# ucuapps/OpenGlue

Hardware: NVIDIA H100
Metric: image-pairs/sec at N=M=2048, d=256, 9 GNN layers, 100 Sinkhorn iters (higher is better)
Workload: dtype fp16x3 (fp16 hi/lo operands with power-of-two tensor scales, 3 products, fp32 accumulate)

## Files before the change

include/openglue_b200.h:

```cpp
#ifndef OPENGLUE_B200_H_
#define OPENGLUE_B200_H_

#include <stdint.h>

#ifdef __cplusplus
extern "C" {
#endif

#define OG_VERSION 100

typedef enum og_status {
  OG_OK = 0,
  OG_EINVAL = -1,
  OG_EUNSUPPORTED = -2,
  OG_ECUDA = -3,
  OG_EWORKSPACE = -4
} og_status;

typedef enum og_precision {
  OG_PREC_FP32 = 0,
  OG_PREC_TF32X3 = 1,
  OG_PREC_FP16X3 = 2
} og_precision;

// ... 74 lines not shown
  const float* R;  int64_t ldr;  int64_t strideR;
  const float* rscale;
  float* Y;  int64_t ldy;  int64_t strideY;
  float* Yt; int64_t ldyt; int64_t strideYt;
} og_linear_args;
int og_linear_fwd(const og_linear_args* args, int precision, void* stream);
int og_linear_tc_fwd(const og_linear_args* args, const float* Whi, const float* Wlo,
                     float* Yhi, float* Ylo, float* Ythi, float* Ytlo, int mode, void* stream);

int og_attention_fwd(const float* q, int64_t ldq, int64_t strideq,
                     const float* k, int64_t ldk, int64_t stridek,
                     const float* v, int64_t ldv, int64_t stridev,
                     float* out, int64_t ldo, int64_t strideo,
                     int batch, int nq, int nk, int num_heads, int head_dim,
                     int precision, void* stream);

int og_attention_tc_fwd(const float* q, int64_t ldq, int64_t strideq,
                        const float* khi, const float* klo, int64_t ldk,
                        const float* vthi, const float* vtlo, int64_t ldvt,
                        float* out, int64_t ldo, int64_t strideo,
                        int batch, int nq, int nk, int num_heads, int head_dim, void* stream);

int og_weight_split_f16(const float* w, const float* bias, int rows, int cols, void* hi16, void* lo16, float* meta, void* stream);
int og_amax(const float* x, int64_t n, float* slot, void* stream);
int og_linear_f16_fwd(const og_linear_args* args, const void* Wh16, const void* Wl16, const float* w_meta, const float* a_amax,
                      float* amax_out, float* scale_out, void* Yh, void* Yl, void* Yth, void* Ytl, int swap_halves, void* stream);
int og_attention_f16_fwd(const float* q, int64_t ldq, int64_t strideq, const float* q_amax,
                         const void* khi, const void* klo, int64_t ldk, const float* k_scale,
                         const void* vthi, const void* vtlo, int64_t ldvt, const float* v_scale,
                         float* out, int64_t ldo, int64_t strideo, float* out_amax,
                         int batch, int nq, int nk, int num_heads, int head_dim, int swap_halves, void* stream);

int64_t og_sinkhorn_workspace_bytes(int batch, int n, int m);
int og_sinkhorn_fwd(const float* S, int64_t lds, int64_t strideS, const float* dustbin,
                    int batch, int n, int m, int iters, float reg,
                    float* scores, void* workspace, int64_t workspace_bytes, void* stream);

int64_t og_sinkhorn_hist_floats(int batch, int n, int m, int iters);
int og_sinkhorn_train_fwd(const float* S, int64_t lds, int64_t strideS, const float* dustbin,
                          int batch, int n, int m, int iters, float reg, float* scores, float* hist,
                          void* workspace, int64_t workspace_bytes, void* stream);
int64_t og_sinkhorn_bwd_workspace_bytes(int batch, int n, int m, int iters);
int og_sinkhorn_bwd(const float* S, int64_t lds, int64_t strideS, const float* dustbin,
                    int batch, int n, int m, int iters, float reg, const float* hist,
                    const float* dscores, float* dS_aug, float* ddustbin,
                    void* workspace, int64_t workspace_bytes, void* stream);

int64_t og_match_workspace_bytes(int batch, int n, int m);
int og_match_fwd(const float* scores, int batch, int n, int m, float threshold,
                 int64_t* matches0, float* mscores0, int64_t* matches1, float* mscores1,
                 void* workspace, int64_t workspace_bytes, void* stream);

enum { OG_GT_PERSPECTIVE = 0, OG_GT_3D_REPROJECTION = 1 };
typedef struct og_gt_transform {
  int32_t type;
  const float* H;
  const float* K0; const float* K1;
  const float* R;  const float* T;
  const float* depth0;
  const float* depth1;
  int32_t depth_is_image;
  int32_t depth0_h, depth0_w, depth1_h, depth1_w;
} og_gt_transform;

int64_t og_gt_matches_workspace_bytes(int batch, int n, int m);
int og_gt_matches_fwd(const float* kpts0, const float* kpts1, int batch, int n, int m, const og_gt_transform* tf,
// ... 83 lines not shown
```

openglue_b200/_cabi.py:

```python
from __future__ import annotations

import ctypes as C
import os
from typing import Optional

import torch

_HERE = os.path.dirname(os.path.abspath(__file__))
LIB_PATH = os.path.join(_HERE, 'libopenglue_b200.so')

OG_OK = 0
OG_PREC_FP32, OG_PREC_TF32X3, OG_PREC_FP16X3 = 0, 1, 2
OG_MAX_HIDDEN = 8
(OG_T_KENC_W, OG_T_KENC_B, OG_T_QKV_W, OG_T_QKV_B, OG_T_FC1_W, OG_T_FC1_B, OG_T_FC2_W, OG_T_FC2_B,
 OG_T_PROJ_W, OG_T_PROJ_B, OG_T_PROJ_RMIX, OG_T_DUSTBIN) = range(12)


class OgConfig(C.Structure):
    _fields_ = [('descriptor_dim', C.c_int32), ('num_heads', C.c_int32), ('num_layers', C.c_int32),
                ('side_info_size', C.c_int32), ('num_hidden', C.c_int32), ('hidden', C.c_int32 * OG_MAX_HIDDEN),
                ('sinkhorn_iters', C.c_int32), ('sinkhorn_reg', C.c_float), ('match_threshold', C.c_float),
                ('precision', C.c_int32), ('no_descriptors', C.c_int32)]


# ... 17 lines not shown
    _fields_ = [('type', C.c_int32), ('H', C.c_void_p), ('K0', C.c_void_p), ('K1', C.c_void_p), ('R', C.c_void_p),
                ('T', C.c_void_p), ('depth0', C.c_void_p), ('depth1', C.c_void_p), ('depth_is_image', C.c_int32),
                ('depth0_h', C.c_int32), ('depth0_w', C.c_int32), ('depth1_h', C.c_int32), ('depth1_w', C.c_int32)]


OG_GT_PERSPECTIVE, OG_GT_3D_REPROJECTION = 0, 1

SYMBOLS = {
    'og_version': (_I, []),
    'og_last_error': (C.c_char_p, []),
    'og_device_info': (_I, [C.POINTER(C.c_int)] * 3),
    'og_packed_weight_floats': (_L, [_CFG]),
    'og_packed_offset': (_L, [_CFG, _I, _I]),
    'og_workspace_bytes': (_L, [_CFG, _I, _I, _I]),
    'og_split_tf32': (_I, [_P, _P, _P, _L, _P]),
    'og_linear_tc_fwd': (_I, [C.POINTER(OgLinearArgs), _P, _P, _P, _P, _P, _P, _I, _P]),
    'og_superglue_forward': (_I, [_CFG, _P, _P, _P, _I, _I, _I, _P, _P, _P, _P, _P, _P, C.POINTER(C.c_float),
                                  _P, _P, _P, _P, _P, _P, _P, _P, _L, _P]),
    'og_superglue_forward_f16': (_I, [_CFG, _P, _P, _P, _P, _P, _P, _I, _I, _I, _P, _P, _P, _P, _P, _P, C.POINTER(C.c_float),
                                      _P, _P, _P, _P, _P, _P, _P, _P, _L, _P]),
    'og_f16_meta_floats': (_L, [_CFG]),
    'og_pack_f16': (_I, [_CFG, _P, _P, _P, _P, _P]),
    'og_weight_split_f16': (_I, [_P, _P, _I, _I, _P, _P, _P, _P]),
    'og_amax': (_I, [_P, _L, _P, _P]),
    'og_linear_f16_fwd': (_I, [C.POINTER(OgLinearArgs), _P, _P, _P, _P, _P, _P, _P, _P, _P, _P, _I, _P]),
    'og_attention_f16_fwd': (_I, [_P, _L, _L, _P, _P, _P, _L, _P, _P, _P, _L, _P, _P, _L, _L, _P, _I, _I, _I, _I, _I, _I, _P]),
    'og_last_forward_launches': (_I, []),
    'og_set_tuning': (_I, [_I, _I]),
    'og_set_fusion': (_I, [_I]),
    'og_linear_fwd': (_I, [C.POINTER(OgLinearArgs), _I, _P]),
    'og_attention_fwd': (_I, [_P, _L, _L, _P, _L, _L, _P, _L, _L, _P, _L, _L, _I, _I, _I, _I, _I, _I, _P]),
    'og_attention_tc_fwd': (_I, [_P, _L, _L, _P, _P, _L, _P, _P, _L, _P, _L, _L, _I, _I, _I, _I, _I, _P]),
    'og_sinkhorn_workspace_bytes': (_L, [_I, _I, _I]),
    'og_sinkhorn_fwd': (_I, [_P, _L, _L, _P, _I, _I, _I, _I, _F, _P, _P, _L, _P]),
    'og_sinkhorn_hist_floats': (_L, [_I, _I, _I, _I]),
    'og_sinkhorn_train_fwd': (_I, [_P, _L, _L, _P, _I, _I, _I, _I, _F, _P, _P, _P, _L, _P]),
    'og_sinkhorn_bwd_workspace_bytes': (_L, [_I, _I, _I, _I]),
    'og_sinkhorn_bwd': (_I, [_P, _L, _L, _P, _I, _I, _I, _I, _F, _P, _P, _P, _P, _P, _L, _P]),
    'og_match_workspace_bytes': (_L, [_I, _I, _I]),
    'og_match_fwd': (_I, [_P, _I, _I, _I, _F, _P, _P, _P, _P, _P, _L, _P]),
    'og_gt_matches_workspace_bytes': (_L, [_I, _I, _I]),
    'og_collate_fwd': (_I, [_P, _P, _P, _P, _P, _I, _P, _I, _I, _P, _I, _I, _I, _I, _I, _P, _P, _P, _P, _P, _P, _P, _P, _P]),
    'og_criterion_workspace_bytes': (_L, [_I]),
    'og_criterion_fwd': (_I, [_P, _P, _P, _I, _I, _I, _P, _P, _F, _P, _L, _P]),
    'og_gt_matches_fwd': (_I, [_P, _P, _I, _I, _I, C.POINTER(OgGtTransform), _P, _P, _P, _L, _P]),
    'og_train_workspace_floats': (_L, [_I]),
    'og_linear_auto_scratch_floats': (_L, [C.POINTER(OgLinearArgs)]),
    'og_linear_auto_fwd': (_I, [C.POINTER(OgLinearArgs), _I, _P, _P]),
    'og_transpose': (_I, [_P, _L, _L, _P, _L, _L, _I, _I, _I, _I, _P]),
    'og_colsum': (_I, [_P, _L, _P, _L, _P, _L, _I, _I, _P, _P, _P]),
    'og_bn_train_fwd': (_I, [_P, _L, _I, _I, _I, _P, _P, _F, _F, _P, _L, _P, _P, _P, _P, _P, _P]),
    'og_bn_train_bwd': (_I, [_P, _L, _P, _L, _I, _I, _I, _P, _P, _P, _P, _L, _P, _P, _P, _P]),
    'og_softmax_rows': (_I, [_P, _L, _L, _I, _P]),
    'og_softmax_bwd_rows': (_I, [_P, _P, _L, _L, _I, _F, _P]),
    'og_axpby': (_I, [_P, _P, _F, _F, _P, _L, _P]),
    'og_sum_batches': (_I, [_P, _I, _I, _I, _P, _L, _I, _P]),
    'og_mix_fwd': (_I, [_P, _P, _P, _P, _L, _I, _P]),
    'og_mix_bwd': (_I, [_P, _P, _P, _P, _L, _I, _P]),
    'og_mix_param_grad': (_I, [_P, _P, _P, _I, _P]),
    'og_kenc_input': (_I, [_P, _P, _I, _I, _F, _F, _P, _P]),
    'og_sp_im2col3x3': (_I, [_P, _I, _I, _I, _I, _P, _P]),
    'og_sp_maxpool2x2': (_I, [_P, _I, _I, _I, _I, _P, _P]),
    'og_row_normalize': (_I, [_P, _L, _I, _I, _F, _P]),
    'og_sp_heat_nms': (_I, [_P, _I, _I, _I, _I, _F, _I, _P, _P]),
    'og_sp_compact': (_I, [_P, _I, _I, _I, _P, _P, _P, _P]),
    'og_sp_select': (_I, [_P, _P, _P, _P, _P, _I, _I, _I, _I, _I, _P, _P, _P]),
# ... 74 lines not shown
```

openglue_b200/csrc/api.cu:

```cuda
#include "common.cuh"
#include "linear_simt.cuh"
#include "linear_sm90.cuh"
#include "attention_simt.cuh"
#include "attention_sm90.cuh"
#include "sinkhorn.cuh"
#include "sinkhorn_bwd.cuh"
#include "match.cuh"
#include "gt_matches.cuh"
#include "criterion.cuh"
#include "collate.cuh"
#include "train_ops.cuh"
#include "superpoint.cuh"
#include "features.cuh"
#include "homography.cuh"
#include "optim.cuh"
#include <math.h>
#include <string.h>
#include <vector>

namespace og {

__global__ void __launch_bounds__(256) kenc_input_kernel(const float* __restrict__ kpts, const float* __restrict__ side,
                                                          int rows, int S, float wm1, float hm1, float* __restrict__ out) {
  const int r = blockIdx.x * blockDim.x + threadIdx.x;
// ... 271 lines not shown
  }
  return linear_simt_launch(*a, st);
}

int og_split_tf32(const float* src, float* hi, float* lo, int64_t n, void* stream) {
  OG_CHECK_ARG(src && hi && lo && n > 0, "split_tf32: bad arguments");
  return OG_LAUNCH(split_tf32_kernel, (unsigned)((n + 255) / 256), 256, 0, (cudaStream_t)stream, src, hi, lo, n);
}

int og_attention_fwd(const float* q, int64_t ldq, int64_t strideq, const float* k, int64_t ldk, int64_t stridek,
                     const float* v, int64_t ldv, int64_t stridev, float* out, int64_t ldo, int64_t strideo,
                     int batch, int nq, int nk, int num_heads, int head_dim, int precision, void* stream) {
  OG_CHECK_ARG(q && k && v && out, "attention: null pointer");
  OG_CHECK_ARG(batch > 0 && nq > 0 && nk > 0 && num_heads > 0 && head_dim > 0, "attention: bad sizes");
  (void)precision;
  AttnArgs a{q, ldq, strideq, k, ldk, stridek, v, ldv, stridev, out, ldo, strideo, batch, nq, nk, num_heads,
             (float)pow((double)head_dim, -0.5)};
  return attention_simt_launch(a, head_dim, (cudaStream_t)stream);
}

int og_attention_tc_fwd(const float* q, int64_t ldq, int64_t strideq, const float* khi, const float* klo, int64_t ldk,
                        const float* vthi, const float* vtlo, int64_t ldvt, float* out, int64_t ldo, int64_t strideo,
                        int batch, int nq, int nk, int num_heads, int head_dim, void* stream) {
  OG_CHECK_ARG(q && khi && klo && vthi && vtlo && out, "attention_tc: null pointer");
  OG_CHECK_ARG(batch > 0 && nq > 0 && nk > 0 && num_heads > 0, "attention_tc: bad sizes");
  if (!attention_tc_eligible(head_dim, ldq, ldk, ldvt, ldo))
    return fail(OG_EUNSUPPORTED, "attention_tc: head_dim in {32, 64} and 16-byte aligned rows required");
  TcAttnArgs a{q, ldq, strideq, out, ldo, strideo, batch, nq, nk, num_heads, num_heads * head_dim,
               (float)pow((double)head_dim, -0.5)};
  return attention_tc_launch(a, khi, klo, ldk, vthi, vtlo, ldvt, head_dim, (cudaStream_t)stream);
}

int64_t og_sinkhorn_workspace_bytes(int batch, int n, int m) { return sinkhorn_workspace_bytes(batch, n, m); }

int og_sinkhorn_fwd(const float* S, int64_t lds, int64_t strideS, const float* dustbin, int batch, int n, int m,
                    int iters, float reg, float* scores, void* workspace, int64_t workspace_bytes, void* stream) {
  OG_CHECK_ARG(S && dustbin && scores && workspace, "sinkhorn: null pointer");
  OG_CHECK_ARG(batch > 0 && n > 0 && m > 0 && iters >= 0 && reg > 0.f, "sinkhorn: bad sizes");
  return sinkhorn_launch(S, lds, strideS, dustbin, batch, n, m, iters, reg, scores, workspace, workspace_bytes,
                         (cudaStream_t)stream);
}

int64_t og_sinkhorn_hist_floats(int batch, int n, int m, int iters) {
  return (batch > 0 && n > 0 && m > 0 && iters >= 0) ? sinkhorn_hist_floats(batch, n, m, iters) : -1;
}

int og_sinkhorn_train_fwd(const float* S, int64_t lds, int64_t strideS, const float* dustbin, int batch, int n, int m,
                          int iters, float reg, float* scores, float* hist, void* workspace, int64_t workspace_bytes, void* stream) {
  OG_CHECK_ARG(S && dustbin && scores && workspace && hist, "sinkhorn_train_fwd: null pointer");
  OG_CHECK_ARG(batch > 0 && n > 0 && m > 0 && iters >= 0 && reg > 0.f, "sinkhorn_train_fwd: bad sizes");
  return sinkhorn_launch(S, lds, strideS, dustbin, batch, n, m, iters, reg, scores, workspace, workspace_bytes, (cudaStream_t)stream,
                         hist, hist + (int64_t)batch * iters * (n + 1));
}

int64_t og_sinkhorn_bwd_workspace_bytes(int batch, int n, int m, int iters) {
  return (batch > 0 && n > 0 && m > 0 && iters >= 0) ? sinkhorn_bwd_workspace_bytes(batch, n, m, iters) : -1;
}

int og_sinkhorn_bwd(const float* S, int64_t lds, int64_t strideS, const float* dustbin, int batch, int n, int m, int iters, float reg,
                    const float* hist, const float* dscores, float* dS_aug, float* ddustbin, void* workspace, int64_t workspace_bytes,
                    void* stream) {
  OG_CHECK_ARG(S && dustbin && hist && dscores && dS_aug && ddustbin && workspace, "sinkhorn_bwd: null pointer");
  OG_CHECK_ARG(batch > 0 && n > 0 && m > 0 && iters >= 0 && reg > 0.f, "sinkhorn_bwd: bad sizes");
  return sinkhorn_bwd_launch(S, lds, strideS, dustbin, batch, n, m, iters, reg, hist, dscores, dS_aug, ddustbin, workspace,
                             workspace_bytes, (cudaStream_t)stream);
}
// ... 595 lines not shown
```

openglue_b200/csrc/sinkhorn.cuh:

```cuda
#pragma once
#include "common.cuh"
#include "tc_common.cuh"
#include <math_constants.h>
#include <algorithm>

namespace og {

struct SinkArgs {
  static constexpr bool kBackward = false;
  const float* S; int64_t lds, strideS;
  const float* dustbin;
  int B, n, m, iters;
  float reg;
  float norm, log_a_last, log_b_last;
  float* scores;
  float* u;
  float* partial;
  unsigned int* barrier;
  int SP, rows_per_strip, mpad;
  float* hist_u;
  float* hist_v;
};

constexpr int SINK_WARPS = 8;
constexpr int64_t SINK_BARRIER_BYTES = 256 * 128;
constexpr int SINK_MAX_COLS = 8192;
constexpr int SINK_MAX_STRIPS = 32;
constexpr float LOG2E_F = 1.4426950408889634f;

__device__ __forceinline__ void grid_barrier(unsigned int* counter, unsigned int target) {
  __syncthreads();
  if (threadIdx.x == 0) {
    __threadfence();
    atomicAdd(counter, 1u);
    unsigned int seen;
    do {
      asm volatile("ld.acquire.gpu.global.u32 %0, [%1];" : "=r"(seen) : "l"(counter) : "memory");
    } while (seen < target);
    __threadfence();
  }
  __syncthreads();
}

typedef unsigned long long f32x2;
__device__ __forceinline__ f32x2 pk2(float x, float y) { f32x2 r; asm("mov.b64 %0, {%1, %2};" : "=l"(r) : "f"(x), "f"(y)); return r; }
__device__ __forceinline__ void upk2(f32x2 v, float& x, float& y) { asm("mov.b64 {%0, %1}, %2;" : "=f"(x), "=f"(y) : "l"(v)); }
#define OG_F32X2_OP(name, expr)                                        \
  __device__ __forceinline__ f32x2 name(f32x2 a, f32x2 b) {            \
    float ax, ay, bx, by; upk2(a, ax, ay); upk2(b, bx, by);            \
    auto op = [](float u, float v) { return expr; };                   \
    return pk2(op(ax, bx), op(ay, by));                                \
  }
// ... 100 lines not shown
        float4 q = (c < m) ? src[idx] : make_float4(0.f, 0.f, 0.f, 0.f);
        if (c < m && c + 3 >= m) {
          if (c + 1 >= m) q.y = 0.f;
          if (c + 2 >= m) q.z = 0.f;
          q.w = 0.f;
        }
        z[k] = q;
      }
    }
    ++consumed;
    __syncwarp();
    const int nxt = row + SLOTS * G;
    if (lane == 0 && nxt < end_real) copy(sl, nxt);
    if (a.reg != 1.0f) {
      const float reg = a.reg;
#pragma unroll
      for (int k = 0; k < V; ++k) {
        z[k].x = __fdiv_rn(z[k].x, reg); z[k].y = __fdiv_rn(z[k].y, reg);
        z[k].z = __fdiv_rn(z[k].z, reg); z[k].w = __fdiv_rn(z[k].w, reg);
      }
    }
  }
};

template <int V, int W, class X>
__device__ __forceinline__ const X* sink_row_exchange(X* xr, X mine, const SinkStrip<V, W>& s, uint32_t& rowpar) {
  X* x = xr + (rowpar * SinkStrip<V, W>::G + s.grp) * W;
  if (s.lane == 0) x[s.sub] = mine;
  asm volatile("bar.sync %0, %1;" ::"r"(1 + s.grp), "n"(W * 32) : "memory");
  rowpar ^= 1u;
  return x;
}

template <int V, int W, class Args, class Update>
__device__ __forceinline__ void sink_column_reduce(const Args& a, const SinkStrip<V, W>& s, float* red, const float4 (&cacc)[V],
                                                   float cacc_m, int k, Update update) {
  const int m = a.m;
  float* myred = red + s.grp * a.mpad;
#pragma unroll
  for (int q = 0; q < V; ++q) {
    const int c = s.c0 + 4 * (s.lane + 32 * q);
    if (c < m) *reinterpret_cast<float4*>(myred + c) = cacc[q];
  }
  __syncthreads();
  if (s.sub == 0 && s.lane == 0) myred[m] = cacc_m;
  __syncthreads();
  const int64_t buf = (int64_t)(k & 1) * a.B * a.SP + (int64_t)s.b * a.SP;
  float* part = a.partial + (buf + s.strip) * a.mpad;
  for (int j = s.tid; j <= m; j += blockDim.x) {
    float sum = 0.f;
#pragma unroll
    for (int w = 0; w < SinkStrip<V, W>::G; ++w) sum += red[w * a.mpad + j];
    part[j] = sum;
  }
  grid_barrier(a.barrier + 32 * s.b, (unsigned int)(k + 1) * (unsigned int)a.SP);
  const float* pb = a.partial + buf * a.mpad;
  for (int j4 = s.tid; 4 * j4 <= m; j4 += blockDim.x) {
    float4 c = make_float4(0.f, 0.f, 0.f, 0.f);
#pragma unroll 8
    for (int sp = 0; sp < a.SP; ++sp) {
      const float4 q = __ldcg(reinterpret_cast<const float4*>(pb + (int64_t)sp * a.mpad) + j4);
      c.x += q.x; c.y += q.y; c.z += q.z; c.w += q.w;
    }
    const float cc[4] = {c.x, c.y, c.z, c.w};
#pragma unroll
    for (int e = 0; e < 4; ++e) {
      const int j = 4 * j4 + e;
      if (j < m) update(j, cc[e]);
      else if (j == m) update(SinkStrip<V, W>::MC, cc[e]);
    }
  }
  __syncthreads();
}

template <int V, int W, int SLOTS>
__global__ void __launch_bounds__(SINK_WARPS * 32, (V <= 8) ? 2 : 1) sinkhorn_kernel(SinkArgs a) {
  extern __shared__ __align__(128) float og_sink_smem[];
  using Strip = SinkStrip<V, W>;
  constexpr int C = Strip::C, MC = Strip::MC, G = Strip::G;
  float* v_s = og_sink_smem;
  float* red = og_sink_smem + MC + 4;
  float* ring = red + G * a.mpad;
  uint64_t* bars = reinterpret_cast<uint64_t*>(ring + SINK_WARPS * SLOTS * C);
  float2* xr = reinterpret_cast<float2*>(bars + SINK_WARPS * SLOTS);
  const Strip s(a);
  const int n = a.n, m = a.m, c0 = s.c0, lane = s.lane, sub = s.sub;
  const float a_reg = expf(a.norm), a_last = expf(a.log_a_last);
  SinkRowRing<V, W, SLOTS, true, SinkArgs> rows(a, s, ring, bars);
  const float dz = rows.dz;

  for (int j = s.tid; j < MC; j += blockDim.x) v_s[j] = (j < m) ? 0.f : -CUDART_INF_F;
  if (s.tid == 0) v_s[MC] = 0.f;
  __syncthreads();

  rows.prime();
  uint32_t rowpar = 0;
  const f32x2 log2e2 = pk2(LOG2E_F, LOG2E_F);
  for (int it = 0; it < a.iters; ++it) {
    f32x2 cacc[2 * V];
#pragma unroll
    for (int k = 0; k < 2 * V; ++k) cacc[k] = 0ull;
    float cacc_m = 0.f;
    const float v_m = v_s[MC];

    for (int row = s.r0 + s.grp; row < s.r1; row += G) {
      float4 q[V];
      rows.take(row, q);
      f32x2 z[2 * V];
#pragma unroll
      for (int k = 0; k < V; ++k) { z[2 * k] = pk2(q[k].x, q[k].y); z[2 * k + 1] = pk2(q[k].z, q[k].w); }
      const float t_m = dz + v_m;
      float mx = (sub == 0) ? t_m : -CUDART_INF_F;
#pragma unroll
      for (int k = 0; k < V; ++k) {
        const ulonglong2 vv = *reinterpret_cast<const ulonglong2*>(v_s + c0 + 4 * (lane + 32 * k));
        z[2 * k] = add2(z[2 * k], vv.x); z[2 * k + 1] = add2(z[2 * k + 1], vv.y);
        float x0, x1, x2, x3; upk2(z[2 * k], x0, x1); upk2(z[2 * k + 1], x2, x3);
        mx = fmaxf(mx, fmaxf(fmaxf(x0, x1), fmaxf(x2, x3)));
      }
      mx = warp_max(mx);
      const float mxs = (mx == -CUDART_INF_F) ? 0.f : mx;
      const f32x2 mxs2 = pk2(mxs, mxs);
      f32x2 sum2a = 0ull, sum2b = 0ull;
#pragma unroll
      for (int k = 0; k < 2 * V; ++k) {
        float x, y; upk2(mul2(sub2(z[k], mxs2), log2e2), x, y);
        z[k] = pk2(ex2_approx(x), ex2_approx(y));
        if (k & 1) sum2b = add2(sum2b, z[k]); else sum2a = add2(sum2a, z[k]);
      }
      float sa, sb; upk2(add2(sum2a, sum2b), sa, sb);
      const float e_m = (sub == 0) ? ex2_approx((t_m - mxs) * LOG2E_F) : 0.f;
      float s_i = warp_sum(sa + sb) + e_m;
      float mxg = mx, f_w = 1.f;
      if (W > 1) {
        const float2* x = sink_row_exchange(xr, make_float2(mx, s_i), s, rowpar);
        float2 p[W];
#pragma unroll
        for (int w2 = 0; w2 < W; ++w2) { p[w2] = x[w2]; mxg = fmaxf(mxg, p[w2].x); }
        s_i = 0.f;
#pragma unroll
        for (int w2 = 0; w2 < W; ++w2) s_i = fmaf(p[w2].y, ex2_approx((p[w2].x - mxg) * LOG2E_F), s_i);
        f_w = ex2_approx((mx - mxg) * LOG2E_F);
      }
      const float w_i = __fdiv_rn((row < n) ? a_reg : a_last, s_i) * f_w;
      if ((it == a.iters - 1 || a.hist_u) && sub == 0 && lane == 0) {
        const float u_i = ((row < n) ? a.norm : a.log_a_last) - (mxg + logf(s_i));
        if (it == a.iters - 1) a.u[(int64_t)s.b * (n + 1) + row] = u_i;
        if (a.hist_u) a.hist_u[((int64_t)s.b * a.iters + it) * (n + 1) + row] = u_i;
      }
      const f32x2 w2 = pk2(w_i, w_i);
#pragma unroll
      for (int k = 0; k < 2 * V; ++k) cacc[k] = fma2(z[k], w2, cacc[k]);
      cacc_m = fmaf(e_m, w_i, cacc_m);
    }
    rows.prime();
    float4 c4[V];
#pragma unroll
    for (int k = 0; k < V; ++k) { upk2(cacc[2 * k], c4[k].x, c4[k].y); upk2(cacc[2 * k + 1], c4[k].z, c4[k].w); }
    sink_column_reduce(a, s, red, c4, cacc_m, it, [&](int j, float c) {
      v_s[j] = ((j < MC) ? a.norm : a.log_b_last) + v_s[j] - logf(c);
    });
    if (a.hist_v && s.strip == 0) {
      float* hv = a.hist_v + ((int64_t)s.b * (a.iters + 1) + it + 1) * (m + 1);
      for (int j = s.tid; j <= m; j += blockDim.x) hv[j] = (j < m) ? v_s[j] : v_s[MC];
    }
  }

  {
    const float v_m = v_s[MC];
    for (int row = s.r0 + s.grp; row < s.r1; row += G) {
      float4 z[V];
      rows.take(row, z);
      float u_i = 0.f;
      if (a.iters > 0) {
        if (lane == 0) u_i = __ldcg(a.u + (int64_t)s.b * (n + 1) + row);
        u_i = __shfl_sync(0xffffffffu, u_i, 0);
      }
      float* out = a.scores + ((int64_t)s.b * (n + 1) + row) * (m + 1);
#pragma unroll
      for (int k = 0; k < V; ++k) {
        const int c = c0 + 4 * (lane + 32 * k);
        if (c < m) {
          const float4 vv = *reinterpret_cast<const float4*>(v_s + c);
          if (c + 0 < m) out[c + 0] = (z[k].x + u_i) + vv.x - a.norm;
          if (c + 1 < m) out[c + 1] = (z[k].y + u_i) + vv.y - a.norm;
          if (c + 2 < m) out[c + 2] = (z[k].z + u_i) + vv.z - a.norm;
          if (c + 3 < m) out[c + 3] = (z[k].w + u_i) + vv.w - a.norm;
        }
      }
      if (sub == 0 && lane == 0) out[m] = (dz + u_i) + v_m - a.norm;
    }
  }
}

struct SinkPlan { int V, W, slots, occ, SP, rows_per_strip, mpad, pairs_per_launch; size_t smem; };

constexpr size_t sinkhorn_smem(bool backward, int V, int W, int slots, int mpad) {
  const int C = 128 * V, G = SINK_WARPS / W, vecs = backward ? 3 : 1;
  const size_t xbytes = backward ? sizeof(float) : sizeof(float2);
  return ((size_t)vecs * (W * C + 4) + (size_t)G * mpad + (size_t)SINK_WARPS * slots * C) * sizeof(float) +
         (size_t)SINK_WARPS * slots * sizeof(uint64_t) + (size_t)2 * G * W * xbytes + 128;
}

inline int sinkhorn_plan(bool backward, int B, int n, int m, SinkPlan* p) {
  const char* who = backward ? "sinkhorn_bwd" : "sinkhorn";
  if (m <= 512)                { p->V = 4;  p->W = 1; p->slots = 2; }
  else if (m <= 1024)          { p->V = 4;  p->W = 2; p->slots = 2; }
  else if (m <= 2048)          { p->V = 8;  p->W = 2; p->slots = 2; }
  else if (m <= 4096)          { p->V = 16; p->W = 2; p->slots = backward ? 1 : 2; }
  else if (m <= SINK_MAX_COLS) { p->V = 16; p->W = 4; p->slots = 1; }
  else return fail(OG_EUNSUPPORTED, "%s: m = %d > %d columns not supported (swap the images)", who, m, SINK_MAX_COLS);
  p->mpad = (int)align_up(m + 1, 4);
  p->smem = sinkhorn_smem(backward, p->V, p->W, p->slots, p->mpad);
  p->occ = (p->V <= 8 && 2 * (p->smem + 1024) <= OG_SMEM_OPTIN_MAX) ? 2 : 1;
  const int sms = device_info().ok ? device_info().sm_count : 132;
  const int ctas = sms * p->occ;
  p->pairs_per_launch = std::min(B < ctas ? B : ctas, (int)(SINK_BARRIER_BYTES / 128));
  int sp = std::min(ctas / p->pairs_per_launch, SINK_MAX_STRIPS);
  const int max_sp = cdiv(n + 1, SINK_WARPS / p->W);
  if (sp > max_sp) sp = max_sp;
  if (sp < 1) sp = 1;
  p->SP = sp;
  p->rows_per_strip = cdiv(n + 1, sp);
  return OG_OK;
}

inline int sinkhorn_check_rows(const char* who, const float* S, int64_t lds, int64_t strideS, int m) {
  if (lds % 4 != 0 || lds < m || !aligned16(S) || strideS % 4 != 0)
    return fail(OG_EINVAL, "%s: S rows must be 16-byte aligned (lds %% 4 == 0, lds >= m)", who);
  return OG_OK;
}

struct SinkConsts { float norm, log_a_last, log_b_last; };
inline SinkConsts sinkhorn_consts(int n, int m) {
  const float norm = -logf((float)(n + m));
  return {norm, norm + (float)log((double)m),
          norm + (float)log((double)n)};
}

template <auto Kernel, int V, int W, int SLOTS, class Args>
inline int sinkhorn_coop_launch(const Args& a, const SinkPlan& p, cudaStream_t stream) {
  constexpr size_t smem_max = sinkhorn_smem(Args::kBackward, V, W, SLOTS, 128 * V * W + 4);
  static_assert(smem_max <= OG_SMEM_OPTIN_MAX, "Sinkhorn kernel: shared memory beyond what one block may opt in to");
  if (const int rc = smem_opt_in<Kernel>((int)smem_max)) return rc;
  return launch(Args::kBackward ? "sinkhorn_bwd_kernel" : "sinkhorn_kernel", Kernel, LaunchAttr::cooperative, dim3(a.B * a.SP),
                dim3(SINK_WARPS * 32), p.smem, stream, a);
}

template <class Launch>
inline int sinkhorn_for_each_launch(const SinkPlan& p, int B, unsigned int* barrier, cudaStream_t stream, Launch&& launch) {
  for (int b0 = 0; b0 < B; b0 += p.pairs_per_launch) {
    const int nb = std::min(p.pairs_per_launch, B - b0);
    OG_CUDA(cudaMemsetAsync(barrier, 0, (size_t)nb * 128, stream));
    if (const int rc = launch(b0, nb)) return rc;
  }
  return OG_OK;
}

inline int64_t sinkhorn_workspace_bytes(int B, int n, int m) {
  SinkPlan p;
  if (sinkhorn_plan(false, B, n, m, &p) != OG_OK) return -1;
  return SINK_BARRIER_BYTES + align_up((int64_t)B * (n + 1) * 4, 256) + align_up(2LL * B * SINK_MAX_STRIPS * p.mpad * 4, 256);
}

inline int sinkhorn_launch(const float* S, int64_t lds, int64_t strideS, const float* dustbin, int B, int n, int m,
                           int iters, float reg, float* scores, void* ws, int64_t ws_bytes, cudaStream_t stream,
                           float* hist_u = nullptr, float* hist_v = nullptr) {
  SinkPlan p;
  if (const int rc = sinkhorn_plan(false, B, n, m, &p)) return rc;
  if (ws_bytes < sinkhorn_workspace_bytes(B, n, m)) return fail(OG_EWORKSPACE, "sinkhorn: workspace too small");
  if (const int rc = sinkhorn_check_rows("sinkhorn", S, lds, strideS, m)) return rc;
  char* w = static_cast<char*>(ws);
  unsigned int* barrier = reinterpret_cast<unsigned int*>(w); w += SINK_BARRIER_BYTES;
  float* u = reinterpret_cast<float*>(w); w += align_up((int64_t)B * (n + 1) * 4, 256);
  float* partial = reinterpret_cast<float*>(w);
  const SinkConsts k = sinkhorn_consts(n, m);
  if (hist_v) OG_CUDA(cudaMemsetAsync(hist_v, 0, (size_t)B * (iters + 1) * (m + 1) * sizeof(float), stream));
  return sinkhorn_for_each_launch(p, B, barrier, stream, [&](int b0, int nb) {
    SinkArgs a;
    a.S = S + (int64_t)b0 * strideS; a.lds = lds; a.strideS = strideS; a.dustbin = dustbin;
    a.B = nb; a.n = n; a.m = m; a.iters = iters; a.reg = reg;
    a.norm = k.norm; a.log_a_last = k.log_a_last; a.log_b_last = k.log_b_last;
    a.scores = scores + (int64_t)b0 * (n + 1) * (m + 1);
    a.u = u; a.partial = partial; a.barrier = barrier;
    a.SP = p.SP; a.rows_per_strip = p.rows_per_strip; a.mpad = p.mpad;
    a.hist_u = hist_u ? hist_u + (int64_t)b0 * iters * (n + 1) : nullptr;
    a.hist_v = hist_v ? hist_v + (int64_t)b0 * (iters + 1) * (m + 1) : nullptr;
    if (p.V == 4 && p.W == 1) return sinkhorn_coop_launch<sinkhorn_kernel<4, 1, 2>, 4, 1, 2>(a, p, stream);
    if (p.V == 4)             return sinkhorn_coop_launch<sinkhorn_kernel<4, 2, 2>, 4, 2, 2>(a, p, stream);
    if (p.V == 8)             return sinkhorn_coop_launch<sinkhorn_kernel<8, 2, 2>, 8, 2, 2>(a, p, stream);
    if (p.W == 2)             return sinkhorn_coop_launch<sinkhorn_kernel<16, 2, 2>, 16, 2, 2>(a, p, stream);
    return sinkhorn_coop_launch<sinkhorn_kernel<16, 4, 1>, 16, 4, 1>(a, p, stream);
  });
}

}
```

Before: 465.4.

## Add resident Sinkhorn kernel holding score rows on-chip with tagged flag exchange

Adds a Sinkhorn forward kernel that keeps each strip's score rows resident in registers and shared memory across all iterations, instead of re-streaming S from global memory every iteration. It also replaces the grid barrier with per-element tagged relaxed stores and polling to reduce and exchange the column potentials. A cost model picks between resident and streaming modes, and an env var and API can turn it off. The risks are spin-wait polling overhead, the assumption that all blocks are co-resident, and extra shared-memory pressure.

New measurement: 484.3, median of 6. 1.04x the previous value.

```diff
diff --git a/include/openglue_b200.h b/include/openglue_b200.h
--- a/include/openglue_b200.h
+++ b/include/openglue_b200.h
@@ -130,6 +130,8 @@
                          int batch, int nq, int nk, int num_heads, int head_dim, int swap_halves, void* stream);
 
 int64_t og_sinkhorn_workspace_bytes(int batch, int n, int m);
+int og_set_sinkhorn_resident(int resident);
+int og_sinkhorn_plan(int batch, int n, int m, int64_t* plan);
 int og_sinkhorn_fwd(const float* S, int64_t lds, int64_t strideS, const float* dustbin,
                     int batch, int n, int m, int iters, float reg,
                     float* scores, void* workspace, int64_t workspace_bytes, void* stream);
diff --git a/openglue_b200/_cabi.py b/openglue_b200/_cabi.py
--- a/openglue_b200/_cabi.py
+++ b/openglue_b200/_cabi.py
@@ -73,6 +73,8 @@
     'og_attention_fwd': (_I, [_P, _L, _L, _P, _L, _L, _P, _L, _L, _P, _L, _L, _I, _I, _I, _I, _I, _I, _P]),
     'og_attention_tc_fwd': (_I, [_P, _L, _L, _P, _P, _L, _P, _P, _L, _P, _L, _L, _I, _I, _I, _I, _I, _P]),
     'og_sinkhorn_workspace_bytes': (_L, [_I, _I, _I]),
+    'og_set_sinkhorn_resident': (_I, [_I]),
+    'og_sinkhorn_plan': (_I, [_I, _I, _I, _P]),
     'og_sinkhorn_fwd': (_I, [_P, _L, _L, _P, _I, _I, _I, _I, _F, _P, _P, _L, _P]),
     'og_sinkhorn_hist_floats': (_L, [_I, _I, _I, _I]),
     'og_sinkhorn_train_fwd': (_I, [_P, _L, _L, _P, _I, _I, _I, _I, _F, _P, _P, _P, _L, _P]),
diff --git a/openglue_b200/csrc/api.cu b/openglue_b200/csrc/api.cu
--- a/openglue_b200/csrc/api.cu
+++ b/openglue_b200/csrc/api.cu
@@ -327,6 +327,27 @@
 }
 
 int64_t og_sinkhorn_workspace_bytes(int batch, int n, int m) { return sinkhorn_workspace_bytes(batch, n, m); }
+
+int og_set_sinkhorn_resident(int resident) {
+  const int prev = sink_resident_mode();
+  if (resident >= 0) sink_resident_mode() = resident ? 1 : 0;
+  return prev;
+}
+
+int og_sinkhorn_plan(int batch, int n, int m, int64_t* plan) {
+  OG_CHECK_ARG(plan, "sinkhorn_plan: null pointer");
+  OG_CHECK_ARG(batch > 0 && n > 0 && m > 0, "sinkhorn_plan: bad sizes");
+  SinkPlan p;
+  const bool resident = sink_resident_mode() && sinkhorn_resident_plan(batch, n, m, &p);
+  if (!resident) {
+    if (const int rc = sinkhorn_plan(false, batch, n, m, &p)) return rc;
+    p.rows_reg = p.rows_smem = 0;
+  }
+  const int64_t v[10] = {resident, p.V, p.W, p.SP, p.rows_per_strip, p.pairs_per_launch, p.rows_reg, p.rows_smem,
+                         (int64_t)p.smem, p.occ};
+  for (int i = 0; i < 10; ++i) plan[i] = v[i];
+  return OG_OK;
+}
 
 int og_sinkhorn_fwd(const float* S, int64_t lds, int64_t strideS, const float* dustbin, int batch, int n, int m,
                     int iters, float reg, float* scores, void* workspace, int64_t workspace_bytes, void* stream) {
diff --git a/openglue_b200/csrc/sinkhorn.cuh b/openglue_b200/csrc/sinkhorn.cuh
--- a/openglue_b200/csrc/sinkhorn.cuh
+++ b/openglue_b200/csrc/sinkhorn.cuh
@@ -18,6 +18,8 @@
   float* partial;
   unsigned int* barrier;
   int SP, rows_per_strip, mpad;
+  int rows_smem;
+  float* vglob;
   float* hist_u;
   float* hist_v;
 };
@@ -184,27 +186,34 @@
   return x;
 }
 
+template <int V, int W, class Args, class Store>
+__device__ __forceinline__ void sink_strip_sums(const Args& a, const SinkStrip<V, W>& s, float* red, const float4 (&cacc)[V],
+                                                float cacc_m, Store store) {
+  const int m = a.m;
+  float* myred = red + s.grp * a.mpad;
+#pragma unroll
+  for (int q = 0; q < V; ++q) {
+    const int c = s.c0 + 4 * (s.lane + 32 * q);
+    if (c < m) *reinterpret_cast<float4*>(myred + c) = cacc[q];
+  }
+  __syncthreads();
+  if (s.sub == 0 && s.lane == 0) myred[m] = cacc_m;
+  __syncthreads();
+  for (int j = s.tid; j <= m; j += blockDim.x) {
+    float sum = 0.f;
+#pragma unroll
+    for (int w = 0; w < SinkStrip<V, W>::G; ++w) sum += red[w * a.mpad + j];
+    store(j, sum);
+  }
+}
+
 template <int V, int W, class Args, class Update>
 __device__ __forceinline__ void sink_column_reduce(const Args& a, const SinkStrip<V, W>& s, float* red, const float4 (&cacc)[V],
                                                    float cacc_m, int k, Update update) {
   const int m = a.m;
-  float* myred = red + s.grp * a.mpad;
-#pragma unroll
-  for (int q = 0; q < V; ++q) {
-    const int c = s.c0 + 4 * (s.lane + 32 * q);
-    if (c < m) *reinterpret_cast<float4*>(myred + c) = cacc[q];
-  }
-  __syncthreads();
-  if (s.sub == 0 && s.lane == 0) myred[m] = cacc_m;
-  __syncthreads();
   const int64_t buf = (int64_t)(k & 1) * a.B * a.SP + (int64_t)s.b * a.SP;
   float* part = a.partial + (buf + s.strip) * a.mpad;
-  for (int j = s.tid; j <= m; j += blockDim.x) {
-    float sum = 0.f;
-#pragma unroll
-    for (int w = 0; w < SinkStrip<V, W>::G; ++w) sum += red[w * a.mpad + j];
-    part[j] = sum;
-  }
+  sink_strip_sums(a, s, red, cacc, cacc_m, [&](int j, float sum) { part[j] = sum; });
   grid_barrier(a.barrier + 32 * s.b, (unsigned int)(k + 1) * (unsigned int)a.SP);
   const float* pb = a.partial + buf * a.mpad;
   for (int j4 = s.tid; 4 * j4 <= m; j4 += blockDim.x) {
@@ -223,6 +232,84 @@
     }
   }
   __syncthreads();
+}
+
+template <int V, int W>
+__device__ __forceinline__ void sink_fwd_row(const SinkArgs& a, const SinkStrip<V, W>& s, const float4 (&q)[V], const float* v_s,
+                                             float v_m, float dz, float a_reg, float a_last, float2* xr, uint32_t& rowpar, int row,
+                                             int it, f32x2 (&cacc)[2 * V], float& cacc_m) {
+  const int n = a.n, c0 = s.c0, lane = s.lane, sub = s.sub;
+  const f32x2 log2e2 = pk2(LOG2E_F, LOG2E_F);
+  f32x2 z[2 * V];
+#pragma unroll
+  for (int k = 0; k < V; ++k) { z[2 * k] = pk2(q[k].x, q[k].y); z[2 * k + 1] = pk2(q[k].z, q[k].w); }
+  const float t_m = dz + v_m;
+  float mx = (sub == 0) ? t_m : -CUDART_INF_F;
+#pragma unroll
+  for (int k = 0; k < V; ++k) {
+    const ulonglong2 vv = *reinterpret_cast<const ulonglong2*>(v_s + c0 + 4 * (lane + 32 * k));
+    z[2 * k] = add2(z[2 * k], vv.x); z[2 * k + 1] = add2(z[2 * k + 1], vv.y);
+    float x0, x1, x2, x3; upk2(z[2 * k], x0, x1); upk2(z[2 * k + 1], x2, x3);
+    mx = fmaxf(mx, fmaxf(fmaxf(x0, x1), fmaxf(x2, x3)));
+  }
+  mx = warp_max(mx);
+  const float mxs = (mx == -CUDART_INF_F) ? 0.f : mx;
+  const f32x2 mxs2 = pk2(mxs, mxs);
+  f32x2 sum2a = 0ull, sum2b = 0ull;
+#pragma unroll
+  for (int k = 0; k < 2 * V; ++k) {
+    float x, y; upk2(mul2(sub2(z[k], mxs2), log2e2), x, y);
+    z[k] = pk2(ex2_approx(x), ex2_approx(y));
+    if (k & 1) sum2b = add2(sum2b, z[k]); else sum2a = add2(sum2a, z[k]);
+  }
+  float sa, sb; upk2(add2(sum2a, sum2b), sa, sb);
+  const float e_m = (sub == 0) ? ex2_approx((t_m - mxs) * LOG2E_F) : 0.f;
+  float s_i = warp_sum(sa + sb) + e_m;
+  float mxg = mx, f_w = 1.f;
+  if (W > 1) {
+    const float2* x = sink_row_exchange(xr, make_float2(mx, s_i), s, rowpar);
+    float2 p[W];
+#pragma unroll
+    for (int w2 = 0; w2 < W; ++w2) { p[w2] = x[w2]; mxg = fmaxf(mxg, p[w2].x); }
+    s_i = 0.f;
+#pragma unroll
+    for (int w2 = 0; w2 < W; ++w2) s_i = fmaf(p[w2].y, ex2_approx((p[w2].x - mxg) * LOG2E_F), s_i);
+    f_w = ex2_approx((mx - mxg) * LOG2E_F);
+  }
+  const float w_i = __fdiv_rn((row < n) ? a_reg : a_last, s_i) * f_w;
+  if ((it == a.iters - 1 || a.hist_u) && sub == 0 && lane == 0) {
+    const float u_i = ((row < n) ? a.norm : a.log_a_last) - (mxg + logf(s_i));
+    if (it == a.iters - 1) a.u[(int64_t)s.b * (n + 1) + row] = u_i;
+    if (a.hist_u) a.hist_u[((int64_t)s.b * a.iters + it) * (n + 1) + row] = u_i;
+  }
+  const f32x2 w2 = pk2(w_i, w_i);
+#pragma unroll
+  for (int k = 0; k < 2 * V; ++k) cacc[k] = fma2(z[k], w2, cacc[k]);
+  cacc_m = fmaf(e_m, w_i, cacc_m);
+}
+
+template <int V, int W>
+__device__ __forceinline__ void sink_fwd_score_row(const SinkArgs& a, const SinkStrip<V, W>& s, const float4 (&z)[V], const float* v_s,
+                                                   float v_m, float dz, int row) {
+  const int n = a.n, m = a.m, c0 = s.c0, lane = s.lane;
+  float u_i = 0.f;
+  if (a.iters > 0) {
+    if (lane == 0) u_i = __ldcg(a.u + (int64_t)s.b * (n + 1) + row);
+    u_i = __shfl_sync(0xffffffffu, u_i, 0);
+  }
+  float* out = a.scores + ((int64_t)s.b * (n + 1) + row) * (m + 1);
+#pragma unroll
+  for (int k = 0; k < V; ++k) {
+    const int c = c0 + 4 * (lane + 32 * k);
+    if (c < m) {
+      const float4 vv = *reinterpret_cast<const float4*>(v_s + c);
+      if (c + 0 < m) out[c + 0] = (z[k].x + u_i) + vv.x - a.norm;
+      if (c + 1 < m) out[c + 1] = (z[k].y + u_i) + vv.y - a.norm;
+      if (c + 2 < m) out[c + 2] = (z[k].z + u_i) + vv.z - a.norm;
+      if (c + 3 < m) out[c + 3] = (z[k].w + u_i) + vv.w - a.norm;
+    }
+  }
+  if (s.sub == 0 && lane == 0) out[m] = (dz + u_i) + v_m - a.norm;
 }
 
 template <int V, int W, int SLOTS>
@@ -236,7 +323,7 @@
   uint64_t* bars = reinterpret_cast<uint64_t*>(ring + SINK_WARPS * SLOTS * C);
   float2* xr = reinterpret_cast<float2*>(bars + SINK_WARPS * SLOTS);
   const Strip s(a);
-  const int n = a.n, m = a.m, c0 = s.c0, lane = s.lane, sub = s.sub;
+  const int m = a.m;
   const float a_reg = expf(a.norm), a_last = expf(a.log_a_last);
   SinkRowRing<V, W, SLOTS, true, SinkArgs> rows(a, s, ring, bars);
   const float dz = rows.dz;
@@ -247,7 +334,6 @@
 
   rows.prime();
   uint32_t rowpar = 0;
-  const f32x2 log2e2 = pk2(LOG2E_F, LOG2E_F);
   for (int it = 0; it < a.iters; ++it) {
     f32x2 cacc[2 * V];
 #pragma unroll
@@ -258,52 +344,7 @@
     for (int row = s.r0 + s.grp; row < s.r1; row += G) {
       float4 q[V];
       rows.take(row, q);
-      f32x2 z[2 * V];
-#pragma unroll
-      for (int k = 0; k < V; ++k) { z[2 * k] = pk2(q[k].x, q[k].y); z[2 * k + 1] = pk2(q[k].z, q[k].w); }
-      const float t_m = dz + v_m;
-      float mx = (sub == 0) ? t_m : -CUDART_INF_F;
-#pragma unroll
-      for (int k = 0; k < V; ++k) {
-        const ulonglong2 vv = *reinterpret_cast<const ulonglong2*>(v_s + c0 + 4 * (lane + 32 * k));
-        z[2 * k] = add2(z[2 * k], vv.x); z[2 * k + 1] = add2(z[2 * k + 1], vv.y);
-        float x0, x1, x2, x3; upk2(z[2 * k], x0, x1); upk2(z[2 * k + 1], x2, x3);
-        mx = fmaxf(mx, fmaxf(fmaxf(x0, x1), fmaxf(x2, x3)));
-      }
-      mx = warp_max(mx);
-      const float mxs = (mx == -CUDART_INF_F) ? 0.f : mx;
-      const f32x2 mxs2 = pk2(mxs, mxs);
-      f32x2 sum2a = 0ull, sum2b = 0ull;
-#pragma unroll
-      for (int k = 0; k < 2 * V; ++k) {
-        float x, y; upk2(mul2(sub2(z[k], mxs2), log2e2), x, y);
-        z[k] = pk2(ex2_approx(x), ex2_approx(y));
-        if (k & 1) sum2b = add2(sum2b, z[k]); else sum2a = add2(sum2a, z[k]);
-      }
-      float sa, sb; upk2(add2(sum2a, sum2b), sa, sb);
-      const float e_m = (sub == 0) ? ex2_approx((t_m - mxs) * LOG2E_F) : 0.f;
-      float s_i = warp_sum(sa + sb) + e_m;
-      float mxg = mx, f_w = 1.f;
-      if (W > 1) {
-        const float2* x = sink_row_exchange(xr, make_float2(mx, s_i), s, rowpar);
-        float2 p[W];
-#pragma unroll
-        for (int w2 = 0; w2 < W; ++w2) { p[w2] = x[w2]; mxg = fmaxf(mxg, p[w2].x); }
-        s_i = 0.f;
-#pragma unroll
-        for (int w2 = 0; w2 < W; ++w2) s_i = fmaf(p[w2].y, ex2_approx((p[w2].x - mxg) * LOG2E_F), s_i);
-        f_w = ex2_approx((mx - mxg) * LOG2E_F);
-      }
-      const float w_i = __fdiv_rn((row < n) ? a_reg : a_last, s_i) * f_w;
-      if ((it == a.iters - 1 || a.hist_u) && sub == 0 && lane == 0) {
-        const float u_i = ((row < n) ? a.norm : a.log_a_last) - (mxg + logf(s_i));
-        if (it == a.iters - 1) a.u[(int64_t)s.b * (n + 1) + row] = u_i;
-        if (a.hist_u) a.hist_u[((int64_t)s.b * a.iters + it) * (n + 1) + row] = u_i;
-      }
-      const f32x2 w2 = pk2(w_i, w_i);
-#pragma unroll
-      for (int k = 0; k < 2 * V; ++k) cacc[k] = fma2(z[k], w2, cacc[k]);
-      cacc_m = fmaf(e_m, w_i, cacc_m);
+      sink_fwd_row(a, s, q, v_s, v_m, dz, a_reg, a_last, xr, rowpar, row, it, cacc, cacc_m);
     }
     rows.prime();
     float4 c4[V];
@@ -318,34 +359,149 @@
     }
   }
 
-  {
+  const float v_m = v_s[MC];
+  for (int row = s.r0 + s.grp; row < s.r1; row += G) {
+    float4 z[V];
+    rows.take(row, z);
+    sink_fwd_score_row(a, s, z, v_s, v_m, dz, row);
+  }
+}
+
+__device__ __forceinline__ void sink_put(uint64_t* p, float x, uint32_t tag) {
+  asm volatile("st.relaxed.gpu.global.b64 [%0], %1;" ::"l"(p), "l"(((uint64_t)tag << 32) | __float_as_uint(x)) : "memory");
+}
+__device__ __forceinline__ uint64_t sink_get(const uint64_t* p) {
+  uint64_t w;
+  asm volatile("ld.relaxed.gpu.global.b64 %0, [%1];" : "=l"(w) : "l"(p) : "memory");
+  return w;
+}
+constexpr int SINK_POLL = 16;
+template <int N, class At>
+__device__ __forceinline__ void sink_take(float (&x)[N], At at, uint32_t tag) {
+  uint64_t w[N];
+#pragma unroll
+  for (int u = 0; u < N; ++u) { const uint64_t* p = at(u); w[u] = p ? sink_get(p) : (uint64_t)tag << 32; }
+  for (;;) {
+    bool ready = true;
+#pragma unroll
+    for (int u = 0; u < N; ++u) ready &= (uint32_t)(w[u] >> 32) == tag;
+    if (ready) break;
+#pragma unroll
+    for (int u = 0; u < N; ++u)
+      if ((uint32_t)(w[u] >> 32) != tag) w[u] = sink_get(at(u));
+  }
+#pragma unroll
+  for (int u = 0; u < N; ++u) x[u] = __uint_as_float((uint32_t)w[u]);
+}
+
+template <int V, int W, int RR>
+__global__ void __launch_bounds__(SINK_WARPS * 32, 1) sinkhorn_resident_kernel(SinkArgs a) {
+  extern __shared__ __align__(128) float og_sink_smem[];
+  using Strip = SinkStrip<V, W>;
+  constexpr int C = Strip::C, MC = Strip::MC, G = Strip::G, NT = SINK_WARPS * 32;
+  float* v_s = og_sink_smem;
+  float* red = v_s + MC + 4;
+  float* ring = red;
+  float* gsum = red + max(G * a.mpad, SINK_WARPS * C);
+  float4* held = reinterpret_cast<float4*>(gsum + NT);
+  uint64_t* bars = reinterpret_cast<uint64_t*>(held + (size_t)SINK_WARPS * a.rows_smem * (C / 4));
+  float2* xr = reinterpret_cast<float2*>(bars + SINK_WARPS);
+  const Strip s(a);
+  const int m = a.m, lane = s.lane;
+  const float a_reg = expf(a.norm), a_last = expf(a.log_a_last);
+  SinkRowRing<V, W, 1, true, SinkArgs> rows(a, s, ring, bars);
+  const float dz = rows.dz;
+  float4* mine = held + (size_t)(s.grp * W + s.sub) * a.rows_smem * (C / 4);
+  uint64_t* vg = reinterpret_cast<uint64_t*>(a.vglob) + (int64_t)s.b * a.mpad;
+
+  for (int j = s.tid; j < MC; j += blockDim.x) v_s[j] = (j < m) ? 0.f : -CUDART_INF_F;
+  if (s.tid == 0) v_s[MC] = 0.f;
+  __syncthreads();
+
+  rows.prime();
+  uint32_t rowpar = 0;
+  float4 zr[RR][V];
+  for (int it = 0; it <= a.iters; ++it) {
+    const bool last = it == a.iters;
+    f32x2 cacc[2 * V];
+#pragma unroll
+    for (int k = 0; k < 2 * V; ++k) cacc[k] = 0ull;
+    float cacc_m = 0.f;
     const float v_m = v_s[MC];
-    for (int row = s.r0 + s.grp; row < s.r1; row += G) {
-      float4 z[V];
-      rows.take(row, z);
-      float u_i = 0.f;
-      if (a.iters > 0) {
-        if (lane == 0) u_i = __ldcg(a.u + (int64_t)s.b * (n + 1) + row);
-        u_i = __shfl_sync(0xffffffffu, u_i, 0);
-      }
-      float* out = a.scores + ((int64_t)s.b * (n + 1) + row) * (m + 1);
-#pragma unroll
-      for (int k = 0; k < V; ++k) {
-        const int c = c0 + 4 * (lane + 32 * k);
-        if (c < m) {
-          const float4 vv = *reinterpret_cast<const float4*>(v_s + c);
-          if (c + 0 < m) out[c + 0] = (z[k].x + u_i) + vv.x - a.norm;
-          if (c + 1 < m) out[c + 1] = (z[k].y + u_i) + vv.y - a.norm;
-          if (c + 2 < m) out[c + 2] = (z[k].z + u_i) + vv.z - a.norm;
-          if (c + 3 < m) out[c + 3] = (z[k].w + u_i) + vv.w - a.norm;
+    auto visit = [&](int row, const float4 (&q)[V]) {
+      if (last) sink_fwd_score_row(a, s, q, v_s, v_m, dz, row);
+      else sink_fwd_row(a, s, q, v_s, v_m, dz, a_reg, a_last, xr, rowpar, row, it, cacc, cacc_m);
+    };
+#pragma unroll
+    for (int k = 0; k < RR; ++k) {
+      const int row = s.r0 + s.grp + k * G;
+      if (row < s.r1) {
+        if (it == 0) rows.take(row, zr[k]);
+        visit(row, zr[k]);
+      }
+    }
+    float4* h = mine;
+    for (int row = s.r0 + s.grp + RR * G; row < s.r1; row += G, h += C / 4) {
+      float4 q[V];
+      if (it == 0) {
+        rows.take(row, q);
+#pragma unroll
+        for (int k = 0; k < V; ++k) h[lane + 32 * k] = q[k];
+      } else {
+#pragma unroll
+        for (int k = 0; k < V; ++k) q[k] = h[lane + 32 * k];
+      }
+      visit(row, q);
+    }
+    if (last) break;
+
+    float4 c4[V];
+#pragma unroll
+    for (int k = 0; k < V; ++k) { upk2(cacc[2 * k], c4[k].x, c4[k].y); upk2(cacc[2 * k + 1], c4[k].z, c4[k].w); }
+    if (it == 0) __syncthreads();
+    const uint32_t tag = it + 1;
+    uint64_t* pt = reinterpret_cast<uint64_t*>(a.partial) + (int64_t)s.b * a.SP * a.mpad;
+    sink_strip_sums(a, s, red, c4, cacc_m, [&](int j, float sum) { sink_put(pt + (int64_t)s.strip * a.mpad + j, sum, tag); });
+    const int S = cdiv(m + 1, a.SP), lo = s.strip * S, NG = S >= NT ? 1 : NT / S;
+    auto publish = [&](int j, float c) {
+      sink_put(vg + j, ((j < m) ? a.norm + v_s[j] : a.log_b_last + v_s[MC]) - logf(c), tag);
+    };
+    for (int i = s.tid; i < S * NG; i += NT) {
+      const int j = lo + i % S;
+      float sum = 0.f;
+      if (j <= m) {
+        for (int sp0 = i / S; sp0 < a.SP; sp0 += SINK_POLL * NG) {
+          float x[SINK_POLL];
+          sink_take<SINK_POLL>(x, [&](int u) { const int sp = sp0 + u * NG; return sp < a.SP ? pt + (int64_t)sp * a.mpad + j : nullptr; }, tag);
+#pragma unroll
+          for (int u = 0; u < SINK_POLL; ++u) sum += x[u];
         }
       }
-      if (sub == 0 && lane == 0) out[m] = (dz + u_i) + v_m - a.norm;
-    }
-  }
-}
-
-struct SinkPlan { int V, W, slots, occ, SP, rows_per_strip, mpad, pairs_per_launch; size_t smem; };
+      if (NG > 1) gsum[i] = sum;
+      else if (j <= m) publish(j, sum);
+    }
+    if (NG > 1) {
+      __syncthreads();
+      for (int i = s.tid; i < S && lo + i <= m; i += NT) {
+        float sum = gsum[i];
+        for (int g = 1; g < NG; ++g) sum += gsum[g * S + i];
+        publish(lo + i, sum);
+      }
+    }
+    for (int j0 = s.tid; j0 <= m; j0 += SINK_POLL * NT) {
+      float x[SINK_POLL];
+      sink_take<SINK_POLL>(x, [&](int u) { const int j = j0 + u * NT; return j <= m ? vg + j : nullptr; }, tag);
+#pragma unroll
+      for (int u = 0; u < SINK_POLL; ++u) {
+        const int j = j0 + u * NT;
+        if (j <= m) v_s[(j < m) ? j : MC] = x[u];
+      }
+    }
+    __syncthreads();
+  }
+}
+
+struct SinkPlan { int V, W, slots, occ, SP, rows_per_strip, mpad, pairs_per_launch; size_t smem; bool resident; int rows_reg, rows_smem; };
 
 constexpr size_t sinkhorn_smem(bool backward, int V, int W, int slots, int mpad) {
   const int C = 128 * V, G = SINK_WARPS / W, vecs = backward ? 3 : 1;
@@ -377,6 +533,41 @@
   return OG_OK;
 }
 
+constexpr size_t sinkhorn_resident_smem(int V, int W, int mpad, int rows_smem) {
+  const int C = 128 * V, G = SINK_WARPS / W;
+  return ((size_t)(W * C + 4) + (size_t)std::max(G * mpad, SINK_WARPS * C) + 4 * SINK_WARPS * 32 +
+          (size_t)SINK_WARPS * rows_smem * C) * sizeof(float) +
+         SINK_WARPS * sizeof(uint64_t) + (size_t)2 * G * W * sizeof(float2) + 128;
+}
+
+inline bool sinkhorn_resident_plan(int B, int n, int m, SinkPlan* p) {
+  if (m > 2048 || sinkhorn_plan(false, B, n, m, p) != OG_OK) return false;
+  const int G = SINK_WARPS / p->W, rr = 24 / p->V, C = 128 * p->V;
+  const int sms = device_info().ok ? device_info().sm_count : 132;
+  const int rs_max = (int)((OG_SMEM_OPTIN_MAX - sinkhorn_resident_smem(p->V, p->W, p->mpad, 0)) / (SINK_WARPS * C * sizeof(float)));
+  const int sp_min = cdiv(n + 1, G * (rr + rs_max));
+  if (2 * sp_min > sms) return false;
+  const int rounds = cdiv(B, std::min(B, sms / sp_min));
+  p->pairs_per_launch = cdiv(B, rounds);
+  const int sp = std::min(sms / p->pairs_per_launch, cdiv(n + 1, G));
+  p->rows_per_strip = cdiv(n + 1, sp);
+  p->SP = cdiv(n + 1, p->rows_per_strip);
+  const int rows_per_warp = cdiv(p->rows_per_strip, G);
+  const double resident_us = rounds * (3.8 + rows_per_warp * (0.4 + 0.0625 * p->V));
+  const double streaming_us = 4.0 * B * (n + 1) * (m + 1) / 2.7e6;
+  if (rounds > 1 && resident_us >= streaming_us) return false;
+  p->rows_reg = rr;
+  p->rows_smem = std::max(0, rows_per_warp - rr);
+  p->smem = sinkhorn_resident_smem(p->V, p->W, p->mpad, p->rows_smem);
+  p->slots = 1; p->occ = 1; p->resident = true;
+  return true;
+}
+
+inline int& sink_resident_mode() {
+  static int v = [] { const char* e = getenv("OG_SINK_RESIDENT"); return e ? (atoi(e) != 0) : 1; }();
+  return v;
+}
+
 inline int sinkhorn_check_rows(const char* who, const float* S, int64_t lds, int64_t strideS, int m) {
   if (lds % 4 != 0 || lds < m || !aligned16(S) || strideS % 4 != 0)
     return fail(OG_EINVAL, "%s: S rows must be 16-byte aligned (lds %% 4 == 0, lds >= m)", who);
@@ -410,16 +601,30 @@
 }
 
 inline int64_t sinkhorn_workspace_bytes(int B, int n, int m) {
-  SinkPlan p;
+  SinkPlan p, r;
   if (sinkhorn_plan(false, B, n, m, &p) != OG_OK) return -1;
-  return SINK_BARRIER_BYTES + align_up((int64_t)B * (n + 1) * 4, 256) + align_up(2LL * B * SINK_MAX_STRIPS * p.mpad * 4, 256);
+  int64_t rows = 2LL * B * SINK_MAX_STRIPS;
+  if (sinkhorn_resident_plan(B, n, m, &r)) rows = std::max<int64_t>(rows, 2LL * (r.SP + 1) * r.pairs_per_launch);
+  return SINK_BARRIER_BYTES + align_up((int64_t)B * (n + 1) * 4, 256) + align_up(rows * p.mpad * 4, 256);
+}
+
+template <int V, int W>
+inline int sinkhorn_resident_launch(const SinkArgs& a, const SinkPlan& p, cudaStream_t stream) {
+  constexpr auto kernel = sinkhorn_resident_kernel<V, W, 24 / V>;
+  if (const int rc = smem_opt_in<kernel>((int)OG_SMEM_OPTIN_MAX)) return rc;
+  return launch("sinkhorn_resident_kernel", kernel, LaunchAttr::cooperative, dim3(a.B * a.SP), dim3(SINK_WARPS * 32), p.smem,
+                stream, a);
 }
 
 inline int sinkhorn_launch(const float* S, int64_t lds, int64_t strideS, const float* dustbin, int B, int n, int m,
                            int iters, float reg, float* scores, void* ws, int64_t ws_bytes, cudaStream_t stream,
                            float* hist_u = nullptr, float* hist_v = nullptr) {
   SinkPlan p;
-  if (const int rc = sinkhorn_plan(false, B, n, m, &p)) return rc;
+  const bool resident = !hist_u && !hist_v && sink_resident_mode() && sinkhorn_resident_plan(B, n, m, &p);
+  if (!resident) {
+    if (const int rc = sinkhorn_plan(false, B, n, m, &p)) return rc;
+    p.resident = false;
+  }
   if (ws_bytes < sinkhorn_workspace_bytes(B, n, m)) return fail(OG_EWORKSPACE, "sinkhorn: workspace too small");
   if (const int rc = sinkhorn_check_rows("sinkhorn", S, lds, strideS, m)) return rc;
   char* w = static_cast<char*>(ws);
@@ -436,8 +641,15 @@
     a.scores = scores + (int64_t)b0 * (n + 1) * (m + 1);
     a.u = u; a.partial = partial; a.barrier = barrier;
     a.SP = p.SP; a.rows_per_strip = p.rows_per_strip; a.mpad = p.mpad;
+    a.rows_smem = p.resident ? p.rows_smem : 0;
+    a.vglob = partial + 2LL * p.pairs_per_launch * p.SP * p.mpad;
+    if (p.resident) OG_CUDA(cudaMemsetAsync(partial, 0, 8LL * (p.SP + 1) * p.pairs_per_launch * p.mpad, stream));
     a.hist_u = hist_u ? hist_u + (int64_t)b0 * iters * (n + 1) : nullptr;
     a.hist_v = hist_v ? hist_v + (int64_t)b0 * (iters + 1) * (m + 1) : nullptr;
+    if (p.resident) {
+      if (p.W == 1) return sinkhorn_resident_launch<4, 1>(a, p, stream);
+      return p.V == 4 ? sinkhorn_resident_launch<4, 2>(a, p, stream) : sinkhorn_resident_launch<8, 2>(a, p, stream);
+    }
     if (p.V == 4 && p.W == 1) return sinkhorn_coop_launch<sinkhorn_kernel<4, 1, 2>, 4, 1, 2>(a, p, stream);
     if (p.V == 4)             return sinkhorn_coop_launch<sinkhorn_kernel<4, 2, 2>, 4, 2, 2>(a, p, stream);
     if (p.V == 8)             return sinkhorn_coop_launch<sinkhorn_kernel<8, 2, 2>, 8, 2, 2>(a, p, stream);
```
